# heheyas/V3D

Measured on AMD Instinct MI355X. Metric: multi-view frames/sec, V3D_512 18-frame 25-step EDM, higher is better.
Workload: dtype bf16; 1 GPU; BASELINE.json configs[1]: V3D_512 random-init SVD-XT weights, 1x18x4x64x64 latent, 25 EulerEDM steps, cfg 4.5 (LinearPredictionGuider), 18-frame VideoDecoder decode to 512x512, one sample per GPU; frames=18, edm_steps=25, parallelism=replica x1, hip_graph=False

## Files before the change

include/v3d_hip.h:

```cpp
#ifndef V3D_HIP_H
#define V3D_HIP_H

#include <stdint.h>

#ifdef __cplusplus
extern "C" {
#endif

#define V3D_ABI_VERSION 9

typedef void* v3d_stream_t;

enum {
    V3D_OK = 0,
    V3D_ERR_ARG = -1,
    V3D_ERR_LAUNCH = -2,
};

int v3d_abi_version(void);
const char* v3d_last_error(void);
int v3d_device_info(int32_t* out4);

enum { V3D_GEMM_LINEAR = 0, V3D_GEMM_CONV3X3 = 1, V3D_GEMM_CONVT3 = 2 };

typedef struct v3d_gemm_args {
    const void* A;
    const void* W;
    void* out;
    const float* bias;
    const float* add;
    const void* res1;
    const void* res2;
// ... 19 lines not shown
    int32_t gn_in_silu;
    int64_t gn_nslots;
    const float* gn_in_table;
    int64_t gn_in_rps;
    int64_t gn_in_rows;
    const void* A2;
    int64_t K1, lda2;
} v3d_gemm_args;

int v3d_gemm(const v3d_gemm_args* args, v3d_stream_t stream);
int v3d_gemm_gn_in_supported(const v3d_gemm_args* args);

int v3d_ff_fused(const void* x, int64_t ldx, const void* W1p, const float* b1, const void* W2p, const float* b2,
                 const void* res1, int64_t ldr1, const void* res2, int64_t ldr2, const float* coef, int64_t coef_rpg,
                 float c_acc, float c_res1, float c_res2, void* out, int64_t ldo, int64_t M, int32_t C, int32_t hidden,
                 v3d_stream_t stream);

int v3d_ln_ff_fused(const void* x, int64_t ldx, float ln_eps, const void* W1p, const float* b1, const void* W2p, const float* b2,
                 const void* res1, int64_t ldr1, const void* res2, int64_t ldr2, const float* coef, int64_t coef_rpg,
                 float c_acc, float c_res1, float c_res2, void* out, int64_t ldo, int64_t M, int32_t C, int32_t hidden,
                 v3d_stream_t stream);
int v3d_ln_proj(const void* x, int64_t ldx, float eps, const void* Wp, const float* bias, void* out, int64_t ldo, void* outT,
                int64_t M, int32_t C, int32_t N, int32_t n_rm, int64_t S, v3d_stream_t stream);
int v3d_sizeof_gemm_args(void);

int v3d_groupnorm_stats(const void* x1, int64_t C1, const void* x2, int64_t C2, float* stats, int64_t nslots,
                        int64_t n_img, int64_t S, int32_t groups, int64_t imgs_per_stat, v3d_stream_t stream);
int v3d_groupnorm_stats_table(const void* x1, int64_t C1, const void* x2, int64_t C2, float* stats, int64_t nslots, uint32_t* tickets,
                              int64_t n_img, int64_t S, int32_t groups, int64_t imgs_per_stat, const float* gamma, const float* beta,
                              double count, float eps, float* table, v3d_stream_t stream);
int v3d_groupnorm_finalize(const float* stats, int64_t nslots, double* sums, int64_t n_stat, int32_t groups,
                           const float* gamma, const float* beta, int64_t C, double count, float eps, float* table,
                           v3d_stream_t stream);
int v3d_groupnorm_apply(const void* x1, int64_t C1, const void* x2, int64_t C2, const float* table, void* out,
                        int64_t n_img, int64_t S, int64_t imgs_per_stat, int32_t silu, v3d_stream_t stream);

int v3d_groupnorm_small_supported(int64_t C1, int64_t C2, int64_t S, int32_t groups, int64_t imgs_per_stat);
int v3d_groupnorm_small(const void* x1, int64_t C1, const void* x2, int64_t C2, const float* gamma, const float* beta, void* out,
                        int64_t n_img, int64_t S, int32_t groups, int64_t imgs_per_stat, float eps, int32_t silu, v3d_stream_t stream);

int v3d_layernorm(const void* x, const float* add, int64_t add_rpg, int64_t add_ld, void* xsum_out,
                  const float* gamma, const float* beta, void* out, int64_t M, int64_t C, float eps,
                  v3d_stream_t stream);

int v3d_attn_spatial(const void* q, int64_t ldq, const void* k, int64_t ldk, const void* vT, void* out,
                     int64_t ldo, int64_t n_img, int64_t S, int32_t heads, float scale, v3d_stream_t stream);
// ... 93 lines not shown
```

v3d_amd/engine/blocks.py:

```python
from __future__ import annotations

import os
from dataclasses import dataclass
from typing import Optional

import torch

from ..ops import GEMM_CONV3X3, GEMM_CONVT3, GemmCall, OpsBase
from .packing import ResPack


@dataclass
class Geo:
    n: int
    B: int
    T: int
    H: int
    W: int

    @property
    def S(self) -> int:
        return self.H * self.W


# ... 10 lines not shown


_GN_EPILOGUE = int(os.environ.get("V3D_GN_EPILOGUE", "1") or 0)


def _gn_producer(ops, n_stat, rps, cout, device, groups=32, level=1, imgs_per_stat=1, consumer_small=False):
    if consumer_small or _GN_EPILOGUE < level or cout % (2 * groups) or rps % 16:
        return None, {}
    st = ops.gn_stats_buffer(n_stat, device, groups, rps=rps, imgs_per_stat=imgs_per_stat)
    return st, dict(gn_stats=st, gn_rps=rps, gn_cpg=cout // groups)


_CONV_GN = os.environ.get("V3D_CONV_GN", "1") not in ("", "0")


def _halo_level(g: "Geo") -> bool:
    return _CONV_GN and g.W in (16, 32, 64)


def _small_norm(ops, g: "Geo", cout, imgs_per_stat=1) -> bool:
    if imgs_per_stat == 1 and _halo_level(g) and cout % 320 == 0:
        return False
    return ops._GN_SMALL and ops.groupnorm_small_supported(cout, 0, g.S, imgs_per_stat)


def conv3x3_gn(ops, x1, x2, norm, w, bias, g: "Geo", *, stats=None, out=None, **epi):
    ga, be, eps = norm
    n, S = g.n, g.S
    if stats is None and not _halo_level(g) and ops.groupnorm_small_fits(x1, x2, S, 1):
        h = ops.groupnorm(x1, x2, ga, be, n, S, eps=eps, silu=True)
        return ops.conv3x3(h, w, bias, n, g.H, g.W, out=out, **epi)
    table = ops.groupnorm_table(x1, x2, ga, be, n, S, eps=eps, stats=stats)
    N = w.shape[-2]
    K = x1.shape[-1] + (0 if x2 is None else x2.shape[-1])
    if _CONV_GN and g.W != 8:
        if out is None:
            out = ops.empty((n * S, N), ops.act_dtype, x1.device)
        call = GemmCall(A=x1, A2=x2, W=w, out=out, M=n * S, N=N, K=K, bias=bias, mode=GEMM_CONV3X3, Hin=g.H, Win=g.W, Hout=g.H, Wout=g.W,
                        gn_in=table, gn_in_rps=S, gn_in_silu=True, **epi)
        if ops.gemm_gn_in_supported(call):
            ops.gemm(call)
            return out
    h = ops.groupnorm(x1, x2, ga, be, n, S, eps=eps, silu=True, table=table)
    return ops.conv3x3(h, w, bias, n, g.H, g.W, out=out, **epi)


def res_spatial(env: Env, g: Geo, p: ResPack, x1: torch.Tensor, x2: Optional[torch.Tensor], *, eps_override=None, out_stats_imgs=0, out=None):
    ops = env.ops
    S = g.S
    epi = {}
    if p.emb_off >= 0:
        epi = dict(add=env.emb_all[:, p.emb_off:], add_rpg=S, add_ld=env.emb_all.stride(0))
    cout = p.w1.shape[-2]
    st2, gkw = _gn_producer(ops, g.n, S, cout, x1.device, consumer_small=_small_norm(ops, g, cout))
    h = conv3x3_gn(ops, x1, x2, p.gn1, p.w1, p.b1, g, **epi, **gkw)
    if p.skip_w is None:
        assert x2 is None
        skip = x1
    else:
        if x2 is None:
            skip = ops.linear(x1, p.skip_w, p.skip_b)
        else:
            c1 = x1.shape[-1]
            skip = ops.linear(x1, p.skip_w[:, :c1], p.skip_b)
            skip = ops.linear(x2, p.skip_w[:, c1:], None, res1=skip)
    if not out_stats_imgs:
        return conv3x3_gn(ops, h, None, p.gn2, p.w2, p.b2, g, stats=st2, res1=skip, out=out)
    st, gkw = _gn_producer(ops, g.n // out_stats_imgs, out_stats_imgs * S, p.w2.shape[-2], x1.device, imgs_per_stat=out_stats_imgs,
                           consumer_small=env.shard is None and _small_norm(ops, g, p.w2.shape[-2], out_stats_imgs))
    return conv3x3_gn(ops, h, None, p.gn2, p.w2, p.b2, g, stats=st2, res1=skip, out=out, **gkw), st


def convt3_gn(ops, x, norm, w, bias, g: "Geo", *, stats=None, **epi):
    ga, be, eps = norm
    n, S, T = g.n, g.S, g.T
    N, K = w.shape[-2], x.shape[-1]
    if stats is None and ops.groupnorm_small_fits(x, None, S, T):
        h = ops.groupnorm(x, None, ga, be, n, S, eps=eps, silu=True, imgs_per_stat=T)
        return ops.convt3(h, w, bias, T, S, **epi)
    table = ops.groupnorm_table(x, None, ga, be, n, S, eps=eps, imgs_per_stat=T, stats=stats)
    tiles = (n * S // 192) * (N // 320) if N % 320 == 0 else 0
    cus = getattr(ops, "cu_count", 256)
    pays = getattr(ops, "always_fuse", False) or (tiles > 0 and tiles * 10 >= -(-tiles // cus) * cus * 9)
    if _CONV_GN and pays:
        out = ops.empty((n * S, N), ops.act_dtype, x.device)
        call = GemmCall(A=x, W=w, out=out, M=n * S, N=N, K=K, bias=bias, mode=GEMM_CONVT3, T=T, S=S, tmin=0, tmax=T - 1,
                        gn_in=table, gn_in_rps=T * S, gn_in_silu=True, **epi)
        if ops.gemm_gn_in_supported(call):
# ... 63 lines not shown
```

v3d_amd/engine/standalone.py:

```python
from __future__ import annotations

import torch

from ..ops import get_ops
from .blocks import Env, Geo, unet_resblock, vae_resblock
from .packing import _Collector, _bf, _f, pack_resblock, pack_svt, pack_vae_resblock, _pack_attnblock

F32 = torch.float32


def _signature(mod):
    return tuple((p.data_ptr(), p._version, str(p.device)) for p in mod.parameters())


def _cached(mod, build):
    sig = _signature(mod)
    hit = mod.__dict__.get("_v3d_standalone")
    if hit is None or hit[0] != sig:
        hit = (sig, build())
        object.__setattr__(mod, "_v3d_standalone", hit)
    return hit[1]


def _rows(ops, x):
    return ops.nchw_to_nhwc_bf16(x.float().contiguous(), 1.0, x.shape[1])


def _nchw(rows, n, H, W, like):
# ... 107 lines not shown
    ops = get_ops()
    B, N, C = x.shape
    dev = x.device

    def build():
        wq, wk, wv = (_bf(m.weight) for m in (at.to_q, at.to_k, at.to_v))
        return wq, wk, wv, pack_linear(at.to_out[0])

    wq, wk, wv, wo = _cached(at, build)
    inner = wq.shape[0]
    if context is not None:
        if context.dim() != 3 or context.shape[0] != B or context.shape[1] != 1:
            raise NotImplementedError("CrossAttention with more than one context token per batch element is not used by V3D / SVD")
        v = ops.linear(_tokens(ops, context), wv)
        o = ops.linear(v, wo[0], wo[1], out_dtype=F32)
        return o[:, None, :].expand(B, N, o.shape[-1]).to(x.dtype).contiguous()
    assert at.dim_head == 64, "attention kernels are specialised for dim_head = 64"
    rows = _tokens(ops, x)
    q, k = ops.linear(rows, wq), ops.linear(rows, wk)
    vT = ops.empty((B, inner, N), ops.act_dtype, dev) if N % 8 == 0 else ops.empty((B, inner, -(-N // 8) * 8), ops.act_dtype, dev)[..., :N]
    ops.gemm(GemmCall(A=wv, W=rows.view(B, N, C), out=vT, M=inner, N=N, K=C, batch=B))
    a = ops.empty((B * N, inner), ops.act_dtype, dev)
    ops.attn_spatial(q, k, vT, a, B, N, at.heads, float(at.scale))
    return ops.linear(a, wo[0], wo[1]).view(B, N, -1).to(x.dtype)


def basic_transformer_block(blk, x, context=None):
    from .packing import pack_norm
    ops = get_ops()
    B, N, C = x.shape
    cur = _tokens(ops, x)

    def ln(norm, rows):
        ga, be, eps = pack_norm(norm)
        out = ops.empty(tuple(rows.shape), ops.act_dtype, rows.device)
        ops.layernorm(rows, ga, be, out, eps)
        return out

    cur = (cross_attention_module(blk.attn1, ln(blk.norm1, cur).view(B, N, C)).reshape(B * N, C).float() + cur.float())
    cur = _tokens(ops, cur)
    cur = (cross_attention_module(blk.attn2, ln(blk.norm2, cur).view(B, N, C), context).reshape(B * N, C).float() + cur.float())
    cur = _tokens(ops, cur)
    cur = feed_forward_module(blk.ff, ln(blk.norm3, cur)).float() + cur.float()
    return cur.view(B, N, C).to(x.dtype)
```

v3d_amd/engine/unet.py:

```python
from __future__ import annotations

import os

from typing import Optional

import torch

from ..ops import GemmCall, get_ops
from .blocks import Env, Geo, unet_resblock
from .packing import SVTPack, UNetPack, cross_attn_pack, round_up

BF, F32 = torch.bfloat16, torch.float32


def _cast_rows_bf16(ops, x2d: torch.Tensor, pad_to: int = 0) -> torch.Tensor:
    n, C = x2d.shape
    return ops.nchw_to_nhwc_bf16(x2d.float().contiguous().reshape(n, C, 1), 1.0, max(pad_to, round_up(C, 8)))


def frame_pos_table(ops, p: SVTPack, B: int, frame_ids) -> torch.Tensor:
    key = (B, tuple(frame_ids))
    tab = p.tables.get(key)
    if tab is None:
        dev = p.proj_in[0].device
        t = torch.tensor(list(frame_ids), dtype=F32, device=dev)
        te = ops.timestep_embedding(t, p.C, p.max_period)
        w0, b0, w2, b2 = p.tpe
        h = ops.silu_add(ops.linear(te, w0, b0, out_dtype=F32))
        tab = ops.linear(h, w2, b2, out_dtype=F32).repeat(B, 1).contiguous()
        p.tables[key] = tab
    return tab

# ... 5 lines not shown
    R = M // G
    assert G * R == M and 2 <= n_ctx <= 32, f"cross-attention: {M} rows / {G} contexts of {n_ctx} tokens (2..32 tokens)"
    QB = max(d for d in range(1, 33) if R % d == 0)
    n2 = ops.empty((M, C), ops.act_dtype, x.device)
    ops.layernorm(x, ga, be, n2, eps)
    q = ops.linear(n2, wq)
    kv = ops.linear(ctx_rows, wkv)
    a = ops.empty((M, C), ops.act_dtype, x.device)
    blk = lambda t: t.view(G, R // QB, QB, C).permute(0, 2, 1, 3)
    tok = lambda t: t.view(G, n_ctx, 1, C).expand(G, n_ctx, R // QB, C)
    ops.attn_temporal(blk(q), tok(kv[:, :C]), tok(kv[:, C:]), blk(a), heads, 0.125)
    return ops.linear(a, wo, bo, res1=x)


def run_svt(env: Env, g: Geo, p: SVTPack, x_in: torch.Tensor) -> torch.Tensor:
    ops = env.ops
    n, S, C, T, B = g.n, g.S, p.C, g.T, g.B
    sh = env.shard
    ctx = env.ctx_all
    ctx_ld = ctx.stride(0) if ctx is not None else 0

    ga, be, eps = p.norm
    h = ops.groupnorm(x_in, None, ga, be, n, S, eps=eps, silu=False)
    x = ops.linear(h, *p.proj_in)

    ga, be, eps = p.s_norm1
    ln_proj = (os.environ.get("V3D_LN_PROJ", "1") not in ("", "0") and p.s_wqkv_fused is not None and C in getattr(ops, "LN_PROJ_WIDTHS", ())
               and S % 128 == 0)
    n1 = None
    if ln_proj:
        qk, vT = ops.ln_proj(x, eps, p.s_wqkv_fused[0], p.s_wqkv_fused[1], 2 * C, S)
    else:
        n1 = ops.empty((n * S, C), ops.act_dtype, x.device)
        ops.layernorm(x, ga, be, n1, eps)
        qk = ops.linear(n1, p.s_wqk)
        vT = ops.empty((n, C, S), ops.act_dtype, x.device) if S % 8 == 0 else ops.empty((n, C, -(-S // 8) * 8), ops.act_dtype, x.device)[..., :S]
        ops.gemm(GemmCall(A=p.s_wv, W=n1.view(n, S, C), out=vT, M=C, N=S, K=C, batch=n))
    a = ops.empty((n * S, C), ops.act_dtype, x.device)
    if os.environ.get("V3D_ATTN_FP8", "0") not in ("", "0") and hasattr(ops, "attn_spatial_fp8") and S % 16 == 0:
        qk8, qk_scales = ops.quant_fp8_tiles(qk, n, S)
        v8, v_scale = ops.quant_fp8_slab(vT, p.heads)
        ops.attn_spatial_fp8(qk8, qk_scales, v8, v_scale, a, n, S, p.heads, 0.125)
    else:
        ops.attn_spatial(qk[:, :C], qk[:, C:], vT, a, n, S, p.heads, 0.125)
    multi = env.ctx_tok is not None
    if multi:
        x = ops.linear(a, p.s_wo[0], p.s_wo[1], res1=x)
        x = cross_attention(ops, x, cross_attn_pack(p, "s"), env.ctx_tok, env.n_ctx, p.heads)
    else:
        x = ops.linear(a, p.s_wo[0], p.s_wo[1], res1=x, add=ctx[:, p.s_ctx_off:], add_rpg=S, add_ld=ctx_ld)
    x_s = feed_forward(ops, x, p.s_ff, res1=x, ln=p.s_norm3)

    frames = range(T) if sh is None else sh.local_frames
    table = frame_pos_table(ops, p, B, frames)
    ga, be, eps = p.t_norm_in
    x_mix = ops.empty((n * S, C), ops.act_dtype, x.device)
    nin = ops.empty((n * S, C), ops.act_dtype, x.device)
    ops.layernorm(x_s, ga, be, nin, eps, add=table, add_rpg=S, add_ld=C, xsum_out=x_mix)
    x_t = feed_forward(ops, nin, p.t_ff_in, res1=x_mix)
    ga, be, eps = p.t_norm1
    ta = ops.empty((B, T, S, C), ops.act_dtype, x.device)
    if sh is None and ln_proj:
        qkv = ops.ln_proj(x_t, eps, p.t_wqkv_fused[0], p.t_wqkv_fused[1], 3 * C, S)[0].view(B, T, S, 3 * C)
        ops.attn_temporal(qkv[..., :C], qkv[..., C:2 * C], qkv[..., 2 * C:], ta, p.heads, 0.125)
    elif sh is None:
        n1 = ops.empty((n * S, C), ops.act_dtype, x.device) if n1 is None else n1
        ops.layernorm(x_t, ga, be, n1, eps)
        qkv = ops.linear(n1, p.t_wqkv).view(B, T, S, 3 * C)
        ops.attn_temporal(qkv[..., :C], qkv[..., C:2 * C], qkv[..., 2 * C:], ta, p.heads, 0.125)
    else:
        n1 = ops.empty((n * S, C), ops.act_dtype, x.device) if n1 is None else n1
        ops.layernorm(x_t, ga, be, n1, eps)
        kv_loc = ops.linear(n1, p.t_wqkv[C:]).view(B, T, S, 2 * C)
        kv, pending = sh.allgather_frames(kv_loc, async_op=True)
        q = ops.linear(n1, p.t_wqkv[:C]).view(B, T, S, C)
        pending.wait()
        ops.attn_temporal(q, kv[..., :C], kv[..., C:], ta, p.heads, 0.125)
    if multi:
        x_t = ops.linear(ta.view(n * S, C), p.t_wo[0], p.t_wo[1], res1=x_t)
        x_t = cross_attention(ops, x_t, cross_attn_pack(p, "t"), env.ctx0_tok, env.n_ctx, p.heads)
    else:
        x_t = ops.linear(ta.view(n * S, C), p.t_wo[0], p.t_wo[1], res1=x_t, add=ctx[n:, p.t_ctx_off:], add_rpg=S * T,
                         add_ld=ctx_ld)
    x = feed_forward(ops, x_t, p.t_ff, res1=x_t, res2=x_s, coef=env.coefs[p.mixer], coef_rpg=S, ln=p.t_norm3)
    return ops.linear(x, p.proj_out[0], p.proj_out[1], res1=x_in)


_FF_FUSED = os.environ.get("V3D_FF_FUSED", "1") not in ("", "0")
_LN_FF = os.environ.get("V3D_LN_FF", "1") not in ("", "0")


def feed_forward(ops, xin, ff, *, res1, res2=None, coef=None, coef_rpg=0, ln=None):
    M, C = xin.shape
    kw = dict(res1=res1)
    if res2 is not None:
        kw.update(res2=res2, coef=coef, coef_rpg=coef_rpg)
    fused = _FF_FUSED and ff.w2_fused is not None and M % 128 == 0 and hasattr(ops, "ff_fused")
    if ln is not None:
        if fused and _LN_FF and ff.w1_ln_fused is not None and hasattr(ops, "ln_ff_fused"):
            out = ops.empty((M, C), ops.act_dtype, xin.device)
            return ops.ln_ff_fused(xin, ff.ln_eps, ff.w1_ln_fused, ff.b1_ln_fused, ff.w2_fused, ff.b2, out, **kw)
        ga, be, eps = ln
        normed = ops.empty((M, C), ops.act_dtype, xin.device)
        ops.layernorm(xin, ga, be, normed, eps)
        xin = normed
    if fused:
        out = ops.empty((M, C), ops.act_dtype, xin.device)
        return ops.ff_fused(xin, ff.w1_fused, ff.b1_fused, ff.w2_fused, ff.b2, out, **kw)
# ... 100 lines not shown
```

v3d_amd/hip.py:

```python
from __future__ import annotations

import ctypes as C
import os
from typing import Optional

import torch

from .ops import GemmCall, OpsBase

_HERE = os.path.dirname(os.path.abspath(__file__))
LIB_PATH = os.environ.get("V3D_HIP_LIB") or os.path.join(_HERE, "lib", "libv3d_hip.so")

ABI_VERSION = 9

c_i64, c_i32, c_f32, c_f64, c_vp = C.c_int64, C.c_int32, C.c_float, C.c_double, C.c_void_p


class _GemmArgs(C.Structure):
    _fields_ = [
        ("A", c_vp), ("W", c_vp), ("out", c_vp), ("bias", c_vp), ("add", c_vp), ("res1", c_vp), ("res2", c_vp),
        ("coef", c_vp),
        ("M", c_i64), ("N", c_i64), ("K", c_i64),
        ("lda", c_i64), ("ldw", c_i64), ("ldo", c_i64), ("ldr1", c_i64), ("ldr2", c_i64),
        ("a_rows", c_i64), ("a_row0", c_i64),
        ("add_rpg", c_i64), ("add_ld", c_i64), ("coef_rpg", c_i64),
        ("c_acc", c_f32), ("c_res1", c_f32), ("c_res2", c_f32),
        ("mode", c_i32), ("geglu", c_i32), ("out_fp32", c_i32),
        ("Hin", c_i32), ("Win", c_i32), ("Hout", c_i32), ("Wout", c_i32), ("stride", c_i32), ("up", c_i32),
        ("T", c_i32), ("tmin", c_i32), ("tmax", c_i32),
        ("S", c_i64),
        ("batch", c_i32), ("pad_mode", c_i32),
        ("sA", c_i64), ("sW", c_i64), ("sO", c_i64),
        ("halo_rows", c_i64),
        ("gn_stats", c_vp), ("gn_rps", c_i64), ("gn_cpg", c_i32), ("gn_in_silu", c_i32),
        ("gn_nslots", c_i64),
        ("gn_in_table", c_vp), ("gn_in_rps", c_i64), ("gn_in_rows", c_i64),
        ("A2", c_vp), ("K1", c_i64), ("lda2", c_i64),
    ]


class GsCamera(C.Structure):
    _fields_ = [("view", c_f32 * 16), ("proj", c_f32 * 16), ("tanfovx", c_f32), ("tanfovy", c_f32), ("bg", c_f32 * 3),
                ("width", c_i32), ("height", c_i32)]


_CAM = C.POINTER(GsCamera)

SIGNATURES = {
    "v3d_abi_version": (c_i32, []),
    "v3d_last_error": (C.c_char_p, []),
    "v3d_device_info": (c_i32, [c_vp]),
    "v3d_gemm": (c_i32, [C.POINTER(_GemmArgs), c_vp]),
    "v3d_sizeof_gemm_args": (c_i32, []),
    "v3d_ff_fused": (c_i32, [c_vp, c_i64, c_vp, c_vp, c_vp, c_vp, c_vp, c_i64, c_vp, c_i64, c_vp, c_i64, c_f32, c_f32, c_f32,
                             c_vp, c_i64, c_i64, c_i32, c_i32, c_vp]),
    "v3d_ln_ff_fused": (c_i32, [c_vp, c_i64, c_f32, c_vp, c_vp, c_vp, c_vp, c_vp, c_i64, c_vp, c_i64, c_vp, c_i64, c_f32, c_f32, c_f32,
                                c_vp, c_i64, c_i64, c_i32, c_i32, c_vp]),
    "v3d_ln_proj": (c_i32, [c_vp, c_i64, c_f32, c_vp, c_vp, c_vp, c_i64, c_vp, c_i64, c_i32, c_i32, c_i32, c_i64, c_vp]),
    "v3d_gemm_gn_in_supported": (c_i32, [C.POINTER(_GemmArgs)]),
    "v3d_groupnorm_stats": (c_i32, [c_vp, c_i64, c_vp, c_i64, c_vp, c_i64, c_i64, c_i64, c_i32, c_i64, c_vp]),
    "v3d_groupnorm_stats_table": (c_i32, [c_vp, c_i64, c_vp, c_i64, c_vp, c_i64, c_vp, c_i64, c_i64, c_i32, c_i64, c_vp, c_vp, C.c_double, C.c_float, c_vp, c_vp]),
    "v3d_groupnorm_finalize": (c_i32, [c_vp, c_i64, c_vp, c_i64, c_i32, c_vp, c_vp, c_i64, c_f64, c_f32, c_vp, c_vp]),
    "v3d_groupnorm_apply": (c_i32, [c_vp, c_i64, c_vp, c_i64, c_vp, c_vp, c_i64, c_i64, c_i64, c_i32, c_vp]),
    "v3d_groupnorm_small_supported": (c_i32, [c_i64, c_i64, c_i64, c_i32, c_i64]),
    "v3d_groupnorm_small": (c_i32, [c_vp, c_i64, c_vp, c_i64, c_vp, c_vp, c_vp, c_i64, c_i64, c_i32, c_i64, c_f32, c_i32, c_vp]),
    "v3d_layernorm": (c_i32, [c_vp, c_vp, c_i64, c_i64, c_vp, c_vp, c_vp, c_vp, c_i64, c_i64, c_f32, c_vp]),
    "v3d_attn_spatial": (c_i32, [c_vp, c_i64, c_vp, c_i64, c_vp, c_vp, c_i64, c_i64, c_i64, c_i32, c_f32, c_vp]),
    "v3d_attn_spatial_ld": (c_i32, [c_vp, c_i64, c_vp, c_i64, c_vp, c_i64, c_vp, c_i64, c_i64, c_i64, c_i32, c_f32, c_vp]),
    "v3d_attn_temporal": (c_i32, [c_vp, c_i64, c_i64, c_i64, c_vp, c_vp, c_i64, c_i64, c_i64, c_vp, c_i64, c_i64,
                                  c_i64, c_i64, c_i32, c_i32, c_i64, c_i32, c_f32, c_vp]),
    "v3d_attn_vae_d512": (c_i32, [c_vp, c_i64, c_vp, c_i64, c_vp, c_vp, c_vp, c_i64, c_i64, c_i64, c_i32, c_f32, c_vp]),
    "v3d_quant_fp8_tiles": (c_i32, [c_vp, c_i64, c_vp, c_i64, c_vp, c_i64, c_i64, c_i32, c_vp]),
    "v3d_quant_fp8_slab": (c_i32, [c_vp, c_vp, c_vp, c_vp, c_i64, c_i64, c_i32, c_vp]),
    "v3d_attn_spatial_fp8": (c_i32, [c_vp, c_i64, c_vp, c_vp, c_vp, c_vp, c_i64, c_i64, c_i64, c_i32, c_f32, c_vp]),
    "v3d_softmax_rows": (c_i32, [c_vp, c_vp, c_i64, c_i64, c_vp]),
    "v3d_timestep_embedding": (c_i32, [c_vp, c_vp, c_i64, c_i32, c_f32, c_vp]),
    "v3d_silu_add": (c_i32, [c_vp, c_vp, c_vp, c_i64, c_vp]),
    "v3d_edm_scalings": (c_i32, [c_vp, c_vp, c_vp, c_vp, c_vp, c_i64, c_vp]),
    "v3d_pack_input": (c_i32, [c_vp, c_vp, c_i64, c_vp, c_i64, c_vp, c_i64, c_i64, c_i64, c_vp]),
    "v3d_pack_input_im2col3x3": (c_i32, [c_vp, c_vp, c_i64, c_vp, c_i64, c_vp, c_i64, c_i32, c_i32, c_i64, c_vp]),
    "v3d_tapsum3x3": (c_i32, [c_vp, c_i64, c_vp, c_vp, c_i64, c_i32, c_i32, c_i32, c_vp]),
# ... 45 lines not shown
    if lib.v3d_sizeof_gemm_args() != C.sizeof(_GemmArgs):
        raise RuntimeError(f"v3d_gemm_args layout mismatch: library {lib.v3d_sizeof_gemm_args()} B vs binding {C.sizeof(_GemmArgs)} B")
    return lib


def _ptr(t: Optional[torch.Tensor]):
    return None if t is None else t.data_ptr()


class HipOps(OpsBase):
    name = "hip"

    def __init__(self, device: Optional[torch.device] = None, lib_path: Optional[str] = None):
        self.lib = load_library(lib_path or LIB_PATH)
        if not torch.cuda.is_available():
            raise RuntimeError("v3d_amd: no HIP device visible (torch.cuda.is_available() is False); the V3D hot path "
                               "has no CPU fallback")
        self.device = torch.device("cuda", torch.cuda.current_device()) if device is None else torch.device(device)
        info = (c_i32 * 4)()
        self._check(self.lib.v3d_device_info(C.cast(info, c_vp)), "v3d_device_info")
        self.cu_count, self.lds_bytes, self.wave_size, self.arch = info[0], info[1], info[2], info[3]
        if self.wave_size != 64:
            raise RuntimeError(f"v3d_amd kernels are wave64 gfx950 code; device reports wave size {self.wave_size}")

    def streamk_timeouts(self) -> int:
        fn = self.lib.v3d_debug_sk_timeouts
        fn.restype, fn.argtypes = C.c_longlong, []
        return int(fn())

    def last_gemm_launch(self) -> dict:
        fn = self.lib.v3d_debug_last_gemm_launch
        fn.restype, fn.argtypes = c_i32, [c_vp]
        o = (C.c_longlong * 8)()
        fn(C.cast(o, c_vp))
        fam, bm, bn, tiles, bpc, sk, tail, cus = (int(v) for v in o)
        slots = max(1, bpc) * max(1, cus)
        tiles_eff = tiles * max(1, sk)
        fill = 1.0 if tail else tiles_eff / (-(-tiles_eff // slots) * slots) if tiles_eff else 0.0
        return {"family": fam, "bm": bm, "bn": bn, "tiles": tiles, "blocks_per_cu": bpc, "splitk": sk, "streamk_tail": tail, "cus": cus, "fill": fill}

    def gemm_plan(self, g: GemmCall) -> dict:
        fn = self.lib.v3d_debug_gemm_plan
        fn.restype, fn.argtypes = c_i32, [C.POINTER(_GemmArgs), c_i32, c_vp, c_vp]
        o = (C.c_longlong * 10)()
        a = self._gemm_args(g)
        self._check(fn(C.byref(a), self.cu_count, None, C.cast(o, c_vp)), "v3d_debug_gemm_plan")
# ... 399 lines not shown
            self._req(t, bf, f"ln_ff.{nm}")
        M, Cc = x.shape
        hidden = w2p.shape[-1]
        self._check(self.lib.v3d_ln_ff_fused(x.data_ptr(), x.stride(0), float(eps), w1p.data_ptr(), b1.data_ptr(), w2p.data_ptr(), b2.data_ptr(),
                                             _ptr(res1), res1.stride(0) if res1 is not None else 0, _ptr(res2),
                                             res2.stride(0) if res2 is not None else 0, _ptr(coef), int(coef_rpg), float(c_acc),
                                             float(c_res1), float(c_res2), out.data_ptr(), out.stride(0), M, Cc, hidden, self._stream()),
                    "v3d_ln_ff_fused")
        return out

    LN_PROJ_WIDTHS = (320,)

    def ln_proj(self, x, eps, wp, bias, n_rm, S):
        bf, f32 = torch.bfloat16, torch.float32
        self._req(x, bf, "ln_proj.x"); self._req_c(wp, bf, "ln_proj.w"); self._req_c(bias, f32, "ln_proj.bias")
        M, Cc = x.shape
        N = wp.shape[0]
        out = self.empty((M, n_rm), bf, x.device) if n_rm else None
        outT = self.empty((M // S, N - n_rm, S), bf, x.device) if n_rm < N else None
        self._check(self.lib.v3d_ln_proj(x.data_ptr(), x.stride(0), float(eps), wp.data_ptr(), bias.data_ptr(), _ptr(out),
                                         n_rm if out is not None else 0, _ptr(outT), M, Cc, N, n_rm, S, self._stream()), "v3d_ln_proj")
        return out, outT

    def heun_step(self, x, den, euler, den2, sigma, next_sigma):
        f32 = torch.float32
        for t, nm in ((x, "x"), (den, "den"), (euler, "euler"), (den2, "den2"), (sigma, "sigma"), (next_sigma, "next")):
            self._req_c(t, f32, f"heun.{nm}")
        out = torch.empty_like(x)
        n = x.shape[0]
        self._check(self.lib.v3d_heun_step(x.data_ptr(), den.data_ptr(), euler.data_ptr(), den2.data_ptr(), sigma.data_ptr(),
                                           next_sigma.data_ptr(), out.data_ptr(), n, x.numel() // n, self._stream()), "v3d_heun_step")
        return out

    def clip_preprocess(self, img, size, patch, antialias, mean, std, kpad):
        self._req_c(img, torch.float32, "clip_preprocess.img")
        B, Cc, H, W = img.shape
        if Cc != 3:
            raise RuntimeError("clip_preprocess: expected 3 channels")
        g = size // patch
        out = self.empty((B * g * g, kpad), torch.bfloat16, img.device)
        m3 = (C.c_float * 3)(*[float(v) for v in mean])
        s3 = (C.c_float * 3)(*[float(v) for v in std])
        self._check(self.lib.v3d_clip_preprocess(img.data_ptr(), B, H, W, size, patch, int(bool(antialias)), C.cast(m3, C.c_void_p),
                                                 C.cast(s3, C.c_void_p), out.data_ptr(), kpad, self._stream()), "v3d_clip_preprocess")
        return out

# ... 214 lines not shown
```

Measured before the change: 12.93 frames/s.

## Add weight-stationary persistent GEMM kernel for 320x320 linears and route large ones

Adds a persistent kernel for N=K=320 linear layers. Each block keeps the full weight slice in VGPR/AGPR registers and streams 16-row A fragments, plus the optional residual, through a multi-stage LDS ring using buffer_load_lds. Linears with bias/add/residual epilogues and at least 73728 rows are routed to it through linear_routed. This removes repeated weight reloads and per-tile launch overhead on the big proj_in/proj_out/wo/skip GEMMs. The cost is very high register use at one block per CU and a narrow shape restriction.

```diff
diff --git a/include/v3d_hip.h b/include/v3d_hip.h
--- a/include/v3d_hip.h
+++ b/include/v3d_hip.h
@@ -7,7 +7,7 @@
 extern "C" {
 #endif
 
-#define V3D_ABI_VERSION 9
+#define V3D_ABI_VERSION 10
 
 typedef void* v3d_stream_t;
 
@@ -73,6 +73,12 @@
                  v3d_stream_t stream);
 int v3d_ln_proj(const void* x, int64_t ldx, float eps, const void* Wp, const float* bias, void* out, int64_t ldo, void* outT,
                 int64_t M, int32_t C, int32_t N, int32_t n_rm, int64_t S, v3d_stream_t stream);
+int v3d_linear_ws(const void* A, int64_t lda, const void* W, int64_t ldw, const float* bias, const float* add, int64_t add_rpg, int64_t add_ld,
+                  const void* res1, int64_t ldr1, float c_acc, float c_res1, void* out, int64_t ldo, int64_t M, int32_t N, int32_t K,
+                  v3d_stream_t stream);
+int v3d_linear_ws_supported(const void* A, int64_t lda, const void* W, int64_t ldw, const float* bias, const float* add, int64_t add_rpg,
+                            int64_t add_ld, const void* res1, int64_t ldr1, const void* out, int64_t ldo, int64_t M, int32_t N, int32_t K,
+                            int32_t out_fp32, int32_t other_epilogue);
 int v3d_sizeof_gemm_args(void);
 
 int v3d_groupnorm_stats(const void* x1, int64_t C1, const void* x2, int64_t C2, float* stats, int64_t nslots,
diff --git a/v3d_amd/csrc/linws.hip b/v3d_amd/csrc/linws.hip
--- /dev/null
+++ b/v3d_amd/csrc/linws.hip
@@ -0,0 +1,298 @@
+#include "gemm_common.h"
+
+namespace {
+
+constexpr int LW_ROWS = 16;
+
+__host__ __device__ __forceinline__ long long lw_first(long long b, long long F, long long G) { return b * F / G; }
+
+__device__ __forceinline__ int lw_swz(int row) { return (0x78 >> (((row >> 2) & 3) * 2)) & 3; }
+
+__device__ __forceinline__ void lw_read_frag(u32x4 (&x)[10], unsigned addr) {
+    asm volatile(
+        "ds_read_b128 %0, %10\n\t"
+        "ds_read_b128 %1, %10 offset:1024\n\t"
+        "ds_read_b128 %2, %10 offset:2048\n\t"
+        "ds_read_b128 %3, %10 offset:3072\n\t"
+        "ds_read_b128 %4, %10 offset:4096\n\t"
+        "ds_read_b128 %5, %10 offset:5120\n\t"
+        "ds_read_b128 %6, %10 offset:6144\n\t"
+        "ds_read_b128 %7, %10 offset:7168\n\t"
+        "ds_read_b128 %8, %10 offset:8192\n\t"
+        "ds_read_b128 %9, %10 offset:9216\n\t"
+        "s_waitcnt lgkmcnt(0)"
+        : "=&v"(x[0]), "=&v"(x[1]), "=&v"(x[2]), "=&v"(x[3]), "=&v"(x[4]), "=&v"(x[5]), "=&v"(x[6]), "=&v"(x[7]), "=&v"(x[8]), "=&v"(x[9])
+        : "v"(addr)
+        : "memory");
+}
+__device__ __forceinline__ void lw_read_res(u32x2 (&r)[5], unsigned a0, unsigned a1, unsigned a2, unsigned a3, unsigned a4) {
+    asm volatile(
+        "ds_read_b64 %0, %5\n\t"
+        "ds_read_b64 %1, %6\n\t"
+        "ds_read_b64 %2, %7\n\t"
+        "ds_read_b64 %3, %8\n\t"
+        "ds_read_b64 %4, %9\n\t"
+        "s_waitcnt lgkmcnt(0)"
+        : "=&v"(r[0]), "=&v"(r[1]), "=&v"(r[2]), "=&v"(r[3]), "=&v"(r[4])
+        : "v"(a0), "v"(a1), "v"(a2), "v"(a3), "v"(a4)
+        : "memory");
+}
+__device__ __forceinline__ void lw_read_rows(u32x4 (&r)[3], unsigned a0, unsigned a1, unsigned a2) {
+    asm volatile(
+        "ds_read_b128 %0, %3\n\t"
+        "ds_read_b128 %1, %4\n\t"
+        "ds_read_b128 %2, %5\n\t"
+        "s_waitcnt lgkmcnt(0)"
+        : "=&v"(r[0]), "=&v"(r[1]), "=&v"(r[2])
+        : "v"(a0), "v"(a1), "v"(a2)
+        : "memory");
+}
+__device__ __forceinline__ void lw_load5(f32x4 (&v)[5], const float* ptr) {
+    asm volatile(
+        "global_load_dwordx4 %0, %5, off\n\t"
+        "global_load_dwordx4 %1, %5, off offset:64\n\t"
+        "global_load_dwordx4 %2, %5, off offset:128\n\t"
+        "global_load_dwordx4 %3, %5, off offset:192\n\t"
+        "global_load_dwordx4 %4, %5, off offset:256\n\t"
+        "s_waitcnt vmcnt(0)"
+        : "=&v"(v[0]), "=&v"(v[1]), "=&v"(v[2]), "=&v"(v[3]), "=&v"(v[4])
+        : "v"(ptr)
+        : "memory");
+}
+__device__ __forceinline__ void lw_tile_consts(const GP& p, long long m0f, long long nw0, int lane, E4Tile<5>& t) {
+    const int nb = (int)nw0 + (lane >> 4) * 4;
+    f32x4 bv[5], av[5];
+#pragma unroll
+    for (int j = 0; j < 5; ++j) bv[j] = av[j] = f32x4{0.f, 0.f, 0.f, 0.f};
+    if (p.bias) lw_load5(bv, p.bias + nb);
+    t.add_grp = p.add ? e4_udiv((unsigned)m0f, (unsigned)p.add_rpg) : 0u;
+    t.add_rem = p.add ? (unsigned)m0f - t.add_grp * (unsigned)p.add_rpg : 0u;
+    if (p.add) lw_load5(av, p.add + (long long)t.add_grp * p.add_ld + nb);
+#pragma unroll
+    for (int j = 0; j < 5; ++j) t.ba[j] = bv[j] + av[j];
+    t.ca = p.c_acc;
+    t.c1 = p.c_res1;
+    t.c2 = p.c_res2;
+    t.coef_grp = t.coef_rem = 0u;
+}
+template <int NF>
+__device__ __forceinline__ void lw_fragment(const GP& p, f32x4 (&acc)[NF], long long m0f, long long nw0, int lane, unsigned char* stage, const unsigned (&res_a)[NF],
+                                            unsigned res_base, const E4Tile<NF>& t) {
+    constexpr int CPRO = NF * 2, NP = 16 * CPRO, SROW = NF * 32 + 16;
+    static_assert(NF == 5, "three row pieces per lane, the third on half a wave");
+    const int fr = lane & 15, fq = (lane >> 4) * 4;
+    const unsigned sbase = lds_addr(stage);
+    const unsigned mine = sbase + (unsigned)(fr * SROW + fq * 2);
+    const bool has1 = p.res1 != nullptr;
+    u32x2 rr[NF];
+#pragma unroll
+    for (int j = 0; j < NF; ++j) rr[j] = u32x2{0u, 0u};
+    if (has1) lw_read_res(rr, res_a[0] + res_base, res_a[1] + res_base, res_a[2] + res_base, res_a[3] + res_base, res_a[4] + res_base);
+#pragma unroll
+    for (int j = 0; j < NF; ++j) {
+        float o[4];
+#pragma unroll
+        for (int r = 0; r < 4; ++r) o[r] = (acc[j][r] + t.ba[j][r]) * t.ca;
+        if (has1) {
+            o[0] += t.c1 * bflo(rr[j][0]); o[1] += t.c1 * bfhi(rr[j][0]); o[2] += t.c1 * bflo(rr[j][1]); o[3] += t.c1 * bfhi(rr[j][1]);
+        }
+        const uint32_t w0 = pack2bf(o[0], o[1]), w1 = pack2bf(o[2], o[3]);
+        e4_lds_write8(mine + j * 32, w0, w1);
+    }
+    unsigned ra[3];
+#pragma unroll
+    for (int k = 0; k < 3; ++k) {
+        int c = k * 64 + lane;
+        if (c >= NP) c = lane;
+        ra[k] = sbase + (unsigned)((c / CPRO) * SROW + (c % CPRO) * 16);
+    }
+    u32x4 sr[3];
+    lw_read_rows(sr, ra[0], ra[1], ra[2]);
+    bf16_t* outz = reinterpret_cast<bf16_t*>(p.out) + m0f * p.ldo + nw0;
+#pragma unroll
+    for (int k = 0; k < 3; ++k) {
+        const int c = k * 64 + lane;
+        if (c < NP) *reinterpret_cast<u32x4*>(outz + (long long)(c / CPRO) * p.ldo + (c % CPRO) * 8) = sr[k];
+    }
+}
+
+template <int C, bool RES>
+__global__ __launch_bounds__(256, 1) void linear_ws_kernel(GP p, int nfrag) {
+    static_assert(C == 320, "four waves x 80 columns x K = 320 resident");
+    constexpr int NK = C / 32;
+    constexpr int NF = C / 64;
+    constexpr int WN = NF * 16;
+    constexpr int FPS = 2;
+    constexpr int APIECES = FPS * NK;
+    constexpr int PPW = (RES ? 2 : 1) * APIECES / 4;
+    constexpr int STAGE_BYTES = (RES ? 2 : 1) * APIECES * 1024;
+    constexpr int NS = RES ? 3 : 6;
+    constexpr int RING = NS * STAGE_BYTES;
+    constexpr int EPI_REGION = LW_ROWS * (NF * 32 + 16);
+    constexpr int STORES = E4Cnt<NF>::STORES;
+    constexpr int WAIT_EARLY = PPW * (NS - 2), WAIT_STEADY = WAIT_EARLY + FPS * STORES * (NS - 1);
+    static_assert(APIECES % 4 == 0 && WAIT_STEADY < 64, "pieces per wave / vmcnt range");
+    static_assert(RING + 4 * EPI_REGION <= 160 * 1024, "LDS budget");
+    __shared__ __attribute__((aligned(1024))) unsigned char lds[RING + 4 * EPI_REGION];
+
+    const int tid = threadIdx.x;
+    const int lane = tid & 63;
+    const int wave = __builtin_amdgcn_readfirstlane(tid >> 6);
+    const long long nw0 = wave * WN;
+    unsigned char* estage = lds + RING + wave * EPI_REGION;
+
+    const long long G = gridDim.x;
+    const long long f0 = lw_first(blockIdx.x, nfrag, G);
+    const int nf = (int)(lw_first((long long)blockIdx.x + 1, nfrag, G) - f0);
+    if (nf <= 0) return;
+    const int nst = (nf + FPS - 1) / FPS;
+
+    u32x4 w[NF][NK];
+    {
+        const bf16_t* wz = p.W + (nw0 + (lane & 15)) * p.ldw + (lane >> 4) * 8;
+#pragma unroll
+        for (int j = 0; j < NF; ++j)
+#pragma unroll
+            for (int ks = 0; ks < NK; ++ks) w[j][ks] = *reinterpret_cast<const u32x4*>(wz + (long long)j * 16 * p.ldw + ks * 32);
+        static_assert(NK == 10, "operand list of the statement below");
+#pragma unroll
+        for (int j = 0; j < NF; ++j) {
+            if (j < 3)
+                asm volatile("" : "+v"(w[j][0]), "+v"(w[j][1]), "+v"(w[j][2]), "+v"(w[j][3]), "+v"(w[j][4]), "+v"(w[j][5]), "+v"(w[j][6]), "+v"(w[j][7]),
+                             "+v"(w[j][8]), "+v"(w[j][9]));
+            else
+                asm volatile("" : "+a"(w[j][0]), "+a"(w[j][1]), "+a"(w[j][2]), "+a"(w[j][3]), "+a"(w[j][4]), "+a"(w[j][5]), "+a"(w[j][6]), "+a"(w[j][7]),
+                             "+a"(w[j][8]), "+a"(w[j][9]));
+        }
+    }
+
+    const bufrsrc_t rsA = make_rsrc(p.A, p.a_bytes);
+    const bufrsrc_t rsR = make_rsrc(RES ? (const void*)p.res1 : (const void*)p.A, RES ? p.a2_bytes : p.a_bytes);
+    const int prow = lane >> 2;
+    const unsigned chunk_b = (unsigned)(((lane & 3) ^ lw_swz(prow)) * 16);
+    const unsigned voffA = (unsigned)(prow * p.lda * 2) + chunk_b;
+    const unsigned voffR = (unsigned)(prow * p.ldr1 * 2) + chunk_b;
+    const int a_frag_b = (int)(p.lda * 2 * LW_ROWS), r_frag_b = (int)(p.ldr1 * 2 * LW_ROWS);
+    auto issue = [&](int st, int slot) __attribute__((always_inline)) {
+#pragma unroll
+        for (int i = 0; i < PPW; ++i) {
+            const int q = wave + 4 * i;
+            const bool res = RES && q >= APIECES;
+            const int qq = res ? q - APIECES : q;
+            const int fh = qq >= NK ? 1 : 0, ks = qq - fh * NK;
+            int fl = st * FPS + fh;
+            fl = fl < nf ? fl : nf - 1;
+            const int so = __builtin_amdgcn_readfirstlane((int)(f0 + fl) * (res ? r_frag_b : a_frag_b) + ks * 64);
+            __builtin_amdgcn_raw_ptr_buffer_load_lds(res ? rsR : rsA, (__attribute__((address_space(3))) void*)(lds + slot * STAGE_BYTES + q * 1024), 16,
+                                                     (int)(res ? voffR : voffA), so, 0, 0);
+        }
+    };
+
+    int lane_e = lane;
+    asm volatile("" : "+v"(lane_e));
+    E4Tile<NF> tc;
+    lw_tile_consts(p, f0 * LW_ROWS, nw0, lane_e, tc);
+
+#pragma unroll
+    for (int st = 0; st < NS - 1; ++st) issue(st, st);
+
+    const unsigned frag_a = lds_addr(lds) + (unsigned)((lane & 15) * 64 + (((lane >> 4) ^ lw_swz(lane & 15)) * 16));
+    unsigned res_a[NF];
+#pragma unroll
+    for (int j = 0; j < NF; ++j) {
+        const int row = lane & 15, bcol = wave * (WN * 2) + j * 32 + (lane >> 4) * 8;
+        res_a[j] = lds_addr(lds) + (unsigned)(APIECES * 1024 + (bcol >> 6) * 1024 + row * 64 + ((((bcol & 63) >> 4) ^ lw_swz(row)) * 16) + (bcol & 15));
+    }
+
+    int slot = 0;
+    for (int t = 0; t < nst; ++t) {
+        if (t >= NS - 1) asm volatile("s_waitcnt vmcnt(%0)" ::"n"(WAIT_STEADY) : "memory");
+        else asm volatile("s_waitcnt vmcnt(%0)" ::"n"(WAIT_EARLY) : "memory");
+        __builtin_amdgcn_s_barrier();
+        __builtin_amdgcn_sched_barrier(0);
+        issue(t + NS - 1, slot == 0 ? NS - 1 : slot - 1);
+        __builtin_amdgcn_sched_barrier(0);
+#pragma unroll
+        for (int fh = 0; fh < FPS; ++fh) {
+            const int fl = t * FPS + fh;
+            if (fl < nf) {
+                const unsigned sbase = (unsigned)(slot * STAGE_BYTES + fh * NK * 1024);
+                u32x4 x[NK];
+                lw_read_frag(x, frag_a + sbase);
+                f32x4 acc[NF];
+#pragma unroll
+                for (int j = 0; j < NF; ++j) acc[j] = f32x4{0.f, 0.f, 0.f, 0.f};
+#pragma unroll
+                for (int ks = 0; ks < NK; ++ks)
+#pragma unroll
+                    for (int j = 0; j < NF; ++j)
+                        acc[j] = __builtin_amdgcn_mfma_f32_16x16x32_bf16(__builtin_bit_cast(bf16x8, w[j][ks]), __builtin_bit_cast(bf16x8, x[ks]), acc[j], 0, 0, 0);
+                const long long m0f = (f0 + fl) * LW_ROWS;
+                if (fl > 0) {
+                    tc.add_rem += LW_ROWS;
+                    if (p.add && tc.add_rem >= (unsigned)p.add_rpg) lw_tile_consts(p, m0f, nw0, lane_e, tc);
+                }
+                lw_fragment<NF>(p, acc, m0f, nw0, lane_e, estage, res_a, sbase, tc);
+            }
+        }
+        slot = (slot + 1 == NS) ? 0 : slot + 1;
+    }
+    asm volatile("s_waitcnt vmcnt(0)" ::: "memory");
+}
+
+struct LwCall {
+    const void* A; int64_t lda; const void* W; int64_t ldw; const float* bias; const float* add; int64_t add_rpg, add_ld;
+    const void* res1; int64_t ldr1; void* out; int64_t ldo; int64_t M; int32_t N, K;
+};
+
+const char* lw_refusal(const LwCall& c, int out_fp32, int other_epilogue) {
+    auto al16 = [](const void* q) { return (reinterpret_cast<uintptr_t>(q) & 15) == 0; };
+    if (!c.A || !c.W || !c.out) return "null pointer";
+    if (c.N != 320 || c.K != 320) return "built for N = K = 320";
+    if (out_fp32) return "bf16 output only";
+    if (other_epilogue) return "res2 / blend coefficients / GEGLU / statistics epilogue are not built";
+    if (c.M <= 0 || c.M % LW_ROWS) return "M must be a positive multiple of 16";
+    if (c.lda < c.K || c.lda % 8 || c.ldw < c.K || c.ldw % 8 || c.ldo < c.N || c.ldo % 8) return "row strides: multiples of 8 elements, >= the row";
+    if (!al16(c.A) || !al16(c.W) || !al16(c.out) || (c.bias && !al16(c.bias))) return "misaligned pointer";
+    if (c.add && (!al16(c.add) || c.add_ld % 4 || c.add_rpg <= 0 || c.add_rpg % 16)) return "add: 16-byte aligned, add_ld % 4 == 0, add_rpg a positive multiple of 16";
+    if (c.res1 && (!al16(c.res1) || c.ldr1 < c.N || c.ldr1 % 8)) return "res1: 16-byte aligned, ldr1 a multiple of 8 elements";
+    const long long lim = 1ll << 31;
+    if (c.M * c.lda * 2 >= lim || (c.res1 && c.M * c.ldr1 * 2 >= lim)) return "operand beyond 2 GiB";
+    return nullptr;
+}
+
+}
+
+extern "C" int v3d_linear_ws_supported(const void* A, int64_t lda, const void* W, int64_t ldw, const float* bias, const float* add, int64_t add_rpg,
+                                       int64_t add_ld, const void* res1, int64_t ldr1, const void* out, int64_t ldo, int64_t M, int32_t N, int32_t K,
+                                       int32_t out_fp32, int32_t other_epilogue) {
+    const LwCall c{A, lda, W, ldw, bias, add, add_rpg, add_ld, res1, ldr1, const_cast<void*>(out), ldo, M, N, K};
+    return lw_refusal(c, out_fp32, other_epilogue) == nullptr ? 1 : 0;
+}
+
+extern "C" int v3d_linear_ws(const void* A, int64_t lda, const void* W, int64_t ldw, const float* bias, const float* add, int64_t add_rpg, int64_t add_ld,
+                             const void* res1, int64_t ldr1, float c_acc, float c_res1, void* out, int64_t ldo, int64_t M, int32_t N, int32_t K,
+                             v3d_stream_t stream) {
+    const LwCall c{A, lda, W, ldw, bias, add, add_rpg, add_ld, res1, ldr1, out, ldo, M, N, K};
+    const char* why = lw_refusal(c, 0, 0);
+    V3D_REQUIRE(why == nullptr, "v3d_linear_ws: %s", why);
+    V3dGemmParams p = {};
+    p.A = (const bf16_t*)A; p.W = (const bf16_t*)W; p.out = out; p.bias = bias; p.add = add; p.res1 = (const bf16_t*)res1;
+    p.M = M; p.N = N; p.K = K; p.lda = lda; p.ldw = ldw; p.ldo = ldo; p.ldr1 = ldr1;
+    p.add_rpg = add ? add_rpg : 0; p.add_ld = add ? add_ld : 0;
+    p.c_acc = c_acc; p.c_res1 = c_res1; p.c_res2 = 0.f;
+    p.a_bytes = (unsigned)(((M - 1) * lda + K) * 2);
+    p.a2_bytes = res1 ? (unsigned)(((M - 1) * ldr1 + N) * 2) : 0u;
+    const long long F = M / LW_ROWS;
+    const int cus = v3d_num_cus();
+    const int grid = (int)(F < cus ? F : cus);
+    if (res1) hipLaunchKernelGGL((linear_ws_kernel<320, true>), dim3(grid), dim3(256), 0, (hipStream_t)stream, p, (int)F);
+    else hipLaunchKernelGGL((linear_ws_kernel<320, false>), dim3(grid), dim3(256), 0, (hipStream_t)stream, p, (int)F);
+    return v3d_check_launch("v3d_linear_ws");
+}
+
+extern "C" int v3d_debug_linear_ws_partition(int64_t F, int32_t G, int64_t* begin) {
+    V3D_REQUIRE(F >= 0 && G > 0 && begin != nullptr, "v3d_debug_linear_ws_partition: bad arguments");
+    for (int b = 0; b <= G; ++b) begin[b] = lw_first(b, F, G);
+    return V3D_OK;
+}
diff --git a/v3d_amd/engine/blocks.py b/v3d_amd/engine/blocks.py
--- a/v3d_amd/engine/blocks.py
+++ b/v3d_amd/engine/blocks.py
@@ -56,6 +56,28 @@
     if imgs_per_stat == 1 and _halo_level(g) and cout % 320 == 0:
         return False
     return ops._GN_SMALL and ops.groupnorm_small_supported(cout, 0, g.S, imgs_per_stat)
+
+
+LINEAR_WS_WIDTH = 320
+LINEAR_WS_CLASSES = frozenset({"br", "bar", "r"})
+LINEAR_WS_MIN_ROWS = 73728
+
+
+def linear_ws_class(bias, add, res1) -> str:
+    return ("b" if bias is not None else "") + ("a" if add is not None else "") + ("r" if res1 is not None else "")
+
+
+def linear_ws_route(M: int, K: int, N: int, cls: str, enabled: bool = True) -> bool:
+    return bool(enabled) and K == LINEAR_WS_WIDTH and N == LINEAR_WS_WIDTH and M >= LINEAR_WS_MIN_ROWS and M % 16 == 0 and cls in LINEAR_WS_CLASSES
+
+
+def linear_routed(ops, x, w, bias=None, **epi):
+    if hasattr(ops, "linear_ws") and set(epi) <= {"add", "add_rpg", "add_ld", "res1"}:
+        cls = linear_ws_class(bias, epi.get("add"), epi.get("res1"))
+        if (linear_ws_route(x.shape[0], x.shape[-1], w.shape[-2], cls, getattr(ops, "linear_ws_enabled", False))
+                and ops.linear_ws_supported(x, w, bias, **epi)):
+            return ops.linear_ws(x, w, bias, **epi)
+    return ops.linear(x, w, bias, **epi)
 
 
 def conv3x3_gn(ops, x1, x2, norm, w, bias, g: "Geo", *, stats=None, out=None, **epi):
@@ -93,11 +115,11 @@
         skip = x1
     else:
         if x2 is None:
-            skip = ops.linear(x1, p.skip_w, p.skip_b)
+            skip = linear_routed(ops, x1, p.skip_w, p.skip_b)
         else:
             c1 = x1.shape[-1]
-            skip = ops.linear(x1, p.skip_w[:, :c1], p.skip_b)
-            skip = ops.linear(x2, p.skip_w[:, c1:], None, res1=skip)
+            skip = linear_routed(ops, x1, p.skip_w[:, :c1], p.skip_b)
+            skip = linear_routed(ops, x2, p.skip_w[:, c1:], None, res1=skip)
     if not out_stats_imgs:
         return conv3x3_gn(ops, h, None, p.gn2, p.w2, p.b2, g, stats=st2, res1=skip, out=out)
     st, gkw = _gn_producer(ops, g.n // out_stats_imgs, out_stats_imgs * S, p.w2.shape[-2], x1.device, imgs_per_stat=out_stats_imgs,
diff --git a/v3d_amd/engine/standalone.py b/v3d_amd/engine/standalone.py
--- a/v3d_amd/engine/standalone.py
+++ b/v3d_amd/engine/standalone.py
@@ -3,7 +3,7 @@
 import torch
 
 from ..ops import get_ops
-from .blocks import Env, Geo, unet_resblock, vae_resblock
+from .blocks import Env, Geo, linear_routed, unet_resblock, vae_resblock
 from .packing import _Collector, _bf, _f, pack_resblock, pack_svt, pack_vae_resblock, _pack_attnblock
 
 F32 = torch.float32
@@ -157,7 +157,7 @@
     ops.gemm(GemmCall(A=wv, W=rows.view(B, N, C), out=vT, M=inner, N=N, K=C, batch=B))
     a = ops.empty((B * N, inner), ops.act_dtype, dev)
     ops.attn_spatial(q, k, vT, a, B, N, at.heads, float(at.scale))
-    return ops.linear(a, wo[0], wo[1]).view(B, N, -1).to(x.dtype)
+    return linear_routed(ops, a, wo[0], wo[1]).view(B, N, -1).to(x.dtype)
 
 
 def basic_transformer_block(blk, x, context=None):
diff --git a/v3d_amd/engine/unet.py b/v3d_amd/engine/unet.py
--- a/v3d_amd/engine/unet.py
+++ b/v3d_amd/engine/unet.py
@@ -7,7 +7,7 @@
 import torch
 
 from ..ops import GemmCall, get_ops
-from .blocks import Env, Geo, unet_resblock
+from .blocks import Env, Geo, linear_routed, unet_resblock
 from .packing import SVTPack, UNetPack, cross_attn_pack, round_up
 
 BF, F32 = torch.bfloat16, torch.float32
@@ -59,7 +59,7 @@
 
     ga, be, eps = p.norm
     h = ops.groupnorm(x_in, None, ga, be, n, S, eps=eps, silu=False)
-    x = ops.linear(h, *p.proj_in)
+    x = linear_routed(ops, h, *p.proj_in)
 
     ga, be, eps = p.s_norm1
     ln_proj = (os.environ.get("V3D_LN_PROJ", "1") not in ("", "0") and p.s_wqkv_fused is not None and C in getattr(ops, "LN_PROJ_WIDTHS", ())
@@ -85,7 +85,7 @@
         x = ops.linear(a, p.s_wo[0], p.s_wo[1], res1=x)
         x = cross_attention(ops, x, cross_attn_pack(p, "s"), env.ctx_tok, env.n_ctx, p.heads)
     else:
-        x = ops.linear(a, p.s_wo[0], p.s_wo[1], res1=x, add=ctx[:, p.s_ctx_off:], add_rpg=S, add_ld=ctx_ld)
+        x = linear_routed(ops, a, p.s_wo[0], p.s_wo[1], res1=x, add=ctx[:, p.s_ctx_off:], add_rpg=S, add_ld=ctx_ld)
     x_s = feed_forward(ops, x, p.s_ff, res1=x, ln=p.s_norm3)
 
     frames = range(T) if sh is None else sh.local_frames
@@ -117,10 +117,10 @@
         x_t = ops.linear(ta.view(n * S, C), p.t_wo[0], p.t_wo[1], res1=x_t)
         x_t = cross_attention(ops, x_t, cross_attn_pack(p, "t"), env.ctx0_tok, env.n_ctx, p.heads)
     else:
-        x_t = ops.linear(ta.view(n * S, C), p.t_wo[0], p.t_wo[1], res1=x_t, add=ctx[n:, p.t_ctx_off:], add_rpg=S * T,
-                         add_ld=ctx_ld)
+        x_t = linear_routed(ops, ta.view(n * S, C), p.t_wo[0], p.t_wo[1], res1=x_t, add=ctx[n:, p.t_ctx_off:], add_rpg=S * T,
+                            add_ld=ctx_ld)
     x = feed_forward(ops, x_t, p.t_ff, res1=x_t, res2=x_s, coef=env.coefs[p.mixer], coef_rpg=S, ln=p.t_norm3)
-    return ops.linear(x, p.proj_out[0], p.proj_out[1], res1=x_in)
+    return linear_routed(ops, x, p.proj_out[0], p.proj_out[1], res1=x_in)
 
 
 _FF_FUSED = os.environ.get("V3D_FF_FUSED", "1") not in ("", "0")
diff --git a/v3d_amd/hip.py b/v3d_amd/hip.py
--- a/v3d_amd/hip.py
+++ b/v3d_amd/hip.py
@@ -11,7 +11,9 @@
 _HERE = os.path.dirname(os.path.abspath(__file__))
 LIB_PATH = os.environ.get("V3D_HIP_LIB") or os.path.join(_HERE, "lib", "libv3d_hip.so")
 
-ABI_VERSION = 9
+ABI_VERSION = 10
+
+_LINEAR_WS = os.environ.get("V3D_LINEAR_WS", "1") not in ("", "0")
 
 c_i64, c_i32, c_f32, c_f64, c_vp = C.c_int64, C.c_int32, C.c_float, C.c_double, C.c_void_p
 
@@ -57,6 +59,8 @@
     "v3d_ln_ff_fused": (c_i32, [c_vp, c_i64, c_f32, c_vp, c_vp, c_vp, c_vp, c_vp, c_i64, c_vp, c_i64, c_vp, c_i64, c_f32, c_f32, c_f32,
                                 c_vp, c_i64, c_i64, c_i32, c_i32, c_vp]),
     "v3d_ln_proj": (c_i32, [c_vp, c_i64, c_f32, c_vp, c_vp, c_vp, c_i64, c_vp, c_i64, c_i32, c_i32, c_i32, c_i64, c_vp]),
+    "v3d_linear_ws": (c_i32, [c_vp, c_i64, c_vp, c_i64, c_vp, c_vp, c_i64, c_i64, c_vp, c_i64, c_f32, c_f32, c_vp, c_i64, c_i64, c_i32, c_i32, c_vp]),
+    "v3d_linear_ws_supported": (c_i32, [c_vp, c_i64, c_vp, c_i64, c_vp, c_vp, c_i64, c_i64, c_vp, c_i64, c_vp, c_i64, c_i64, c_i32, c_i32, c_i32, c_i32]),
     "v3d_gemm_gn_in_supported": (c_i32, [C.POINTER(_GemmArgs)]),
     "v3d_groupnorm_stats": (c_i32, [c_vp, c_i64, c_vp, c_i64, c_vp, c_i64, c_i64, c_i64, c_i32, c_i64, c_vp]),
     "v3d_groupnorm_stats_table": (c_i32, [c_vp, c_i64, c_vp, c_i64, c_vp, c_i64, c_vp, c_i64, c_i64, c_i32, c_i64, c_vp, c_vp, C.c_double, C.c_float, c_vp, c_vp]),
@@ -148,6 +152,7 @@
         self.cu_count, self.lds_bytes, self.wave_size, self.arch = info[0], info[1], info[2], info[3]
         if self.wave_size != 64:
             raise RuntimeError(f"v3d_amd kernels are wave64 gfx950 code; device reports wave size {self.wave_size}")
+        self.linear_ws_enabled = _LINEAR_WS
 
     def streamk_timeouts(self) -> int:
         fn = self.lib.v3d_debug_sk_timeouts
@@ -593,6 +598,47 @@
                                          n_rm if out is not None else 0, _ptr(outT), M, Cc, N, n_rm, S, self._stream()), "v3d_ln_proj")
         return out, outT
 
+    def _linear_ws_call(self, x, w, bias, out, add, add_rpg, add_ld, res1):
+        bf, f32 = torch.bfloat16, torch.float32
+        self._req(x, bf, "linear_ws.x"); self._req(w, bf, "linear_ws.w")
+        if bias is not None:
+            self._req_c(bias, f32, "linear_ws.bias")
+        if add is not None:
+            self._req(add, f32, "linear_ws.add")
+        if res1 is not None:
+            self._req(res1, bf, "linear_ws.res1")
+        M, K = x.shape
+        N = w.shape[-2]
+        return (x.data_ptr(), x.stride(0), w.data_ptr(), w.stride(-2), _ptr(bias), _ptr(add), add_rpg if add is not None else 0,
+                add_ld if add is not None else 0, _ptr(res1), 0 if res1 is None else res1.stride(0)), \
+               ((x.data_ptr() & ~15) if out is None else out.data_ptr(), N if out is None else out.stride(0), M, N, K)
+
+    def linear_ws_supported(self, x, w, bias=None, *, out=None, add=None, add_rpg=0, add_ld=0, res1=None, out_dtype=None, other_epilogue=False) -> bool:
+        if x.dim() != 2 or w.dim() != 2 or x.dtype != torch.bfloat16 or w.dtype != torch.bfloat16 or x.stride(-1) != 1 or w.stride(-1) != 1:
+            return False
+        fp32 = (out.dtype if out is not None else (out_dtype or self.act_dtype)) == torch.float32
+        if out is not None and (out.dim() != 2 or out.stride(-1) != 1 or tuple(out.shape) != (x.shape[0], w.shape[0])):
+            return False
+        if res1 is not None and (res1.dim() != 2 or res1.stride(-1) != 1 or res1.dtype != torch.bfloat16):
+            return False
+        a, b = self._linear_ws_call(x, w, bias, out, add, add_rpg, add_ld, res1)
+        return bool(self.lib.v3d_linear_ws_supported(*a, *b, int(fp32), int(bool(other_epilogue))))
+
+    def linear_ws(self, x, w, bias=None, *, out=None, add=None, add_rpg=0, add_ld=0, res1=None, c_acc=1.0, c_res1=1.0):
+        if out is None:
+            out = self.empty((x.shape[0], w.shape[-2]), torch.bfloat16, x.device)
+        self._req(out, torch.bfloat16, "linear_ws.out")
+        a, b = self._linear_ws_call(x, w, bias, out, add, add_rpg, add_ld, res1)
+        self._check(self.lib.v3d_linear_ws(*a, float(c_acc), float(c_res1), *b, self._stream()), "v3d_linear_ws")
+        return out
+
+    def linear_ws_partition(self, F: int, G: int):
+        fn = self.lib.v3d_debug_linear_ws_partition
+        fn.restype, fn.argtypes = c_i32, [c_i64, c_i32, c_vp]
+        o = (C.c_int64 * (G + 1))()
+        self._check(fn(F, G, C.cast(o, c_vp)), "v3d_debug_linear_ws_partition")
+        return list(o)
+
     def heun_step(self, x, den, euler, den2, sigma, next_sigma):
         f32 = torch.float32
         for t, nm in ((x, "x"), (den, "den"), (euler, "euler"), (den2, "den2"), (sigma, "sigma"), (next_sigma, "next")):
```

Result: no change. 12.96 frames/s, median of 6 (+0.2%).
